# kuwt/edge_alignment

Measured on NVIDIA B200. Metric: frame-pair alignments/sec at 640x480, higher is better.
Workload: dtype f32+f64

## Files before the change

edge_alignment_b200/csrc/ea_preprocess.cu:

```cuda
#include <cstdlib>

#include "ea_internal.h"

namespace {

__device__ __forceinline__ int reflect101(int i, int n) {
  if (n == 1) return 0;
  while (i < 0 || i >= n) i = (i < 0) ? -i : 2 * n - 2 - i;
  return i;
}

template <typename D>
__global__ void __launch_bounds__(256) k_pyr_down(const uint8_t* __restrict__ src_bgr, const D* __restrict__ src_depth,
                                                  size_t src_frame_stride_px, const int32_t* __restrict__ src_slots,
                                                  uint8_t* __restrict__ dst_bgr, D* __restrict__ dst_depth,
                                                  const int32_t* __restrict__ dst_slots, int sw, int sh) {
  const int dw = sw >> 1, dh = sh >> 1;
  const int f = blockIdx.y;
  const size_t sbase = (src_slots ? size_t(src_slots[f]) : size_t(f)) * src_frame_stride_px;
  const size_t dbase = size_t(dst_slots[f]) * size_t(dw) * dh;
  for (int i = blockIdx.x * blockDim.x + threadIdx.x; i < dw * dh; i += gridDim.x * blockDim.x) {
    const int x = i % dw, y = i / dw;
    const uint8_t* p = src_bgr + (sbase + size_t(2 * y) * sw + 2 * x) * 3;
    const uint8_t* q = p + size_t(sw) * 3;
// ... 274 lines not shown
  const D* dep = depth + (src_slots ? size_t(src_slots[f]) : size_t(f)) * frame_stride_px;
  uint2* out = reinterpret_cast<uint2*>(pts + size_t(slot) * cap);
  const int nw = h * words;
  const int per = (nw + CP_THREADS - 1) / CP_THREADS;
  const int tid = threadIdx.x, lane = tid & 31, warp = tid >> 5;
  const int b = tid * per, e = min(b + per, nw);
  int cnt = 0;
  for (int i = b; i < e; ++i) cnt += __popc(bits[i]);
  int incl = cnt;
#pragma unroll
  for (int o = 1; o < 32; o <<= 1) { const int t = __shfl_up_sync(0xffffffffu, incl, o); if (lane >= o) incl += t; }
  if (lane == 31) warp_sums[warp] = incl;
  __syncthreads();
  if (warp == 0) {
    int v = warp_sums[lane];
    int s = v;
#pragma unroll
    for (int o = 1; o < 32; o <<= 1) { const int t = __shfl_up_sync(0xffffffffu, s, o); if (lane >= o) s += t; }
    warp_sums[lane] = s - v;
    if (lane == 31) total_s = s;
  }
  __syncthreads();
  int rank = warp_sums[warp] + incl - cnt;
  for (int i = b; i < e; ++i) {
    unsigned m = bits[i];
    const int y = i / words, xb = (i % words) * 32;
    while (m) {
      const int bit = __ffs(m) - 1;
      m &= m - 1;
      const int x = xb + bit;
      if (rank < cap) {
        float dz = float(dep[size_t(y) * w + x]);
        if (zero_to_one && dz == 0.0f) dz = depth_one;
        out[rank] = ea_pack_pixel_point(unsigned(x), unsigned(y), dz);
      }
      ++rank;
    }
  }
  if (tid == 0) {
    n_pts[slot * EA_MAX_LEVELS + level] = min(total_s, cap);
    overflow[slot * EA_MAX_LEVELS + level] = total_s > cap ? 1 : 0;
  }
}

__device__ __forceinline__ unsigned long long median3_bits64(unsigned long long a, unsigned long long b, unsigned long long c) {
  const unsigned long long s0 = a ^ b ^ c, s1 = (a & b) | (c & (a ^ b));
  const unsigned long long A0 = s0, B0 = s0 >> 1, C0 = s0 >> 2, A1 = s1, B1 = s1 >> 1, C1 = s1 >> 2;
  const unsigned long long lo = A0 ^ B0 ^ C0, carry = (A0 & B0) | (C0 & (A0 ^ B0));
  const unsigned long long t = A1 ^ B1, u = A1 & B1, v = C1 ^ carry, wv = C1 & carry;
  const unsigned long long m0 = t ^ v, tv = t & v;
  const unsigned long long ge1 = u | wv | tv, eq2 = u & wv;
  const unsigned long long m_ge3 = eq2 | (ge1 & m0);
  const unsigned long long m_eq2 = ge1 & ~eq2 & ~m0;
  return m_ge3 | (m_eq2 & lo);
}
__device__ __forceinline__ unsigned long long row_field64(const uint32_t* __restrict__ row, int wi, int words, int w) {
  const unsigned word = row[wi];
  const int nvalid = min(32, w - 32 * wi);
  const unsigned left = (wi > 0) ? (row[wi - 1] >> 31) : (word & 1u);
  unsigned right;
  if (nvalid == 32 && wi + 1 < words) right = row[wi + 1] & 1u;
  else right = (word >> (nvalid - 1)) & 1u;
  return (static_cast<unsigned long long>(word) << 1) | left | (static_cast<unsigned long long>(right) << (nvalid + 1));
}
__global__ void __launch_bounds__(256) k_median_bits(const __grid_constant__ EaPrepArgs A) {
  const int level = blockIdx.z;
  const EaPrepLevel& L = A.lv[level];
  const int idx = blockIdx.x * blockDim.x + threadIdx.x;
  if (idx >= L.h * L.words) return;
  const int slot = A.slots[blockIdx.y];
  const uint32_t* bits = L.edge_bits + size_t(slot) * L.h * L.words;
  const int y = idx / L.words, wi = idx % L.words;
  const unsigned long long f0 = row_field64(bits + size_t(max(y - 1, 0)) * L.words, wi, L.words, L.w);
  const unsigned long long f1 = row_field64(bits + size_t(y) * L.words, wi, L.words, L.w);
  const unsigned long long f2 = row_field64(bits + size_t(min(y + 1, L.h - 1)) * L.words, wi, L.words, L.w);
  const int nvalid = min(32, L.w - 32 * wi);
  unsigned m = unsigned(median3_bits64(f0, f1, f2));
  if (nvalid < 32) m &= (1u << nvalid) - 1u;
  L.med_bits[size_t(slot) * L.h * L.words + idx] = m;
}

#define DT_HV 62587
#define DT_DG 89738
#define DT_INF 0x3FFFFFFF
#define DT_DISTMAX (0xFFFFFFFFu - 89738u)

template <int P, bool BACKWARD>
__device__ __forceinline__ void dt_row_scan(int (&d)[P], const int (&cval)[P], int lane, int warp, int n_warps, int par,
                                            int (*tot)[32], int (*first)[32], int& left_bnd, int& right_bnd) {
  int dl[P];
  int run = DT_INF;
#pragma unroll
  for (int kk = 0; kk < P; ++kk) {
    const int k = BACKWARD ? (P - 1 - kk) : kk;
    run = min(cval[k], run + DT_HV);
    dl[k] = run;
  }
  const int pos = BACKWARD ? (31 - lane) : lane;
  const int stepP = DT_HV * P;
  int e = min(run, DT_INF) - stepP * pos;
#pragma unroll
  for (int o = 1; o < 32; o <<= 1) {
    const int t = BACKWARD ? __shfl_down_sync(0xffffffffu, e, o) : __shfl_up_sync(0xffffffffu, e, o);
    if (pos >= o) e = min(e, t);
  }
  const int out = e + stepP * pos;
  int carry_local = BACKWARD ? __shfl_down_sync(0xffffffffu, out, 1) : __shfl_up_sync(0xffffffffu, out, 1);
  if (pos == 0) carry_local = DT_INF;
  const int Lw = __shfl_sync(0xffffffffu, out, BACKWARD ? 0 : 31);
  const int f0 = __shfl_sync(0xffffffffu, BACKWARD ? dl[P - 1] : dl[0], BACKWARD ? 31 : 0);
  if (lane == 0) { tot[par][warp] = min(Lw, DT_INF); first[par][warp] = min(f0, DT_INF); }
  __syncthreads();
  const int wpos = BACKWARD ? (n_warps - 1 - warp) : warp;
  const int stepW = stepP * 32;
  int cand = DT_INF;
  if (lane < wpos) {
    const int src = BACKWARD ? (n_warps - 1 - lane) : lane;
    cand = tot[par][src] + stepW * (wpos - 1 - lane);
  }
  const int cw = min(__reduce_min_sync(0xffffffffu, cand), DT_INF);
#pragma unroll
  for (int kk = 0; kk < P; ++kk) {
    const int k = BACKWARD ? (P - 1 - kk) : kk;
    const int v = min(min(dl[k], carry_local + DT_HV * (kk + 1)), cw + DT_HV * (pos * P + kk + 1));
    d[k] = min(v, DT_INF);
  }
  const int out_w = min(min(Lw, cw + stepW), DT_INF);
  const int dn = BACKWARD ? warp - 1 : warp + 1;
  const int dn_first = (dn >= 0 && dn < n_warps) ? min(first[par][dn], out_w + DT_HV) : DT_INF;
  if (BACKWARD) { right_bnd = cw; left_bnd = dn_first; }
  else { left_bnd = cw; right_bnd = dn_first; }
}

template <int P, typename T>
__device__ __forceinline__ void dt_store_row(T* __restrict__ row, int x0, int w, const T (&v)[P], bool vec_ok) {
  if (vec_ok && x0 + P <= w) {
#pragma unroll
    for (int k = 0; k < P; k += 4) *reinterpret_cast<int4*>(row + x0 + k) = *reinterpret_cast<const int4*>(&v[k]);
  } else {
#pragma unroll
    for (int k = 0; k < P; ++k) if (x0 + k < w) row[x0 + k] = v[k];
  }
}
template <int P>
__device__ __forceinline__ void dt_load_row(const int* __restrict__ row, int x0, int w, int (&v)[P], bool vec_ok) {
  if (vec_ok && x0 + P <= w) {
#pragma unroll
    for (int k = 0; k < P; k += 4) *reinterpret_cast<int4*>(&v[k]) = *reinterpret_cast<const int4*>(row + x0 + k);
  } else {
#pragma unroll
    for (int k = 0; k < P; ++k) v[k] = (x0 + k < w) ? row[x0 + k] : DT_INF;
  }
}

template <int P>
__global__ void __launch_bounds__(1024) k_chamfer_dt(const __grid_constant__ EaPrepArgs A) {
  __shared__ int tot[2][32], first[2][32];
  __shared__ unsigned red[2][32];
  const int level = blockIdx.y;
  const EaPrepLevel& L = A.lv[level];
  const int w = L.w, h = L.h, words = L.words;
  const int slot = A.slots[blockIdx.x];
  const uint32_t* bits = (A.use_median ? L.med_bits : L.edge_bits) + size_t(slot) * h * words;
  float* gf = ea_dt_origin(L, slot);
  int* gi = reinterpret_cast<int*>(gf);
  const int pitch = L.dt_pitch;
  const int tid = threadIdx.x, lane = tid & 31, warp = tid >> 5;
  const int n_warps = ((w + P - 1) / P + 31) / 32;
  const bool warp_on = warp < n_warps;
  const int x0 = tid * P;
  const bool vec_ok = (P % 4 == 0) && ((w & 3) == 0);
  int d[P];
#pragma unroll
  for (int k = 0; k < P; ++k) d[k] = DT_INF;
  int left_bnd = DT_INF, right_bnd = DT_INF;
  int par = 0;
  unsigned ebits_next = (warp_on && x0 < w) ? bits[x0 >> 5] : 0u;
  for (int y = 0; y < h; ++y, par ^= 1) {
    if (!warp_on) { __syncthreads(); continue; }
    const unsigned ebits = ebits_next >> (x0 & 31);
    if (x0 < w && y + 1 < h) ebits_next = bits[size_t(y + 1) * words + (x0 >> 5)];
    int pl = __shfl_up_sync(0xffffffffu, d[P - 1], 1);
    int pr = __shfl_down_sync(0xffffffffu, d[0], 1);
    if (lane == 0) pl = left_bnd;
    if (lane == 31) pr = right_bnd;
    int cval[P];
#pragma unroll
    for (int k = 0; k < P; ++k) {
      const int a = (k == 0) ? pl : d[k - 1];
      const int c = (k == P - 1) ? pr : d[k + 1];
      int v = min(min(a, c) + DT_DG, d[k] + DT_HV);
      if ((ebits >> k) & 1u) v = 0;
      if (x0 + k >= w) v = DT_INF;
      cval[k] = min(v, DT_INF);
    }
    dt_row_scan<P, false>(d, cval, lane, warp, n_warps, par, tot, first, left_bnd, right_bnd);
#pragma unroll
    for (int k = 0; k < P; ++k) if (x0 + k >= w) d[k] = DT_INF;
    if (x0 < w) dt_store_row<P, int>(gi + size_t(y) * pitch, x0, w, d, vec_ok);
  }
#pragma unroll
  for (int k = 0; k < P; ++k) d[k] = DT_INF;
  left_bnd = DT_INF; right_bnd = DT_INF;
  unsigned vmax = 0, vmin = 0xFFFFFFFFu;
  int t_next[P];
#pragma unroll
  for (int k = 0; k < P; ++k) t_next[k] = DT_INF;
  if (warp_on && x0 < w) dt_load_row<P>(gi + size_t(h - 1) * pitch, x0, w, t_next, vec_ok);
  for (int y = h - 1; y >= 0; --y, par ^= 1) {
    if (!warp_on) { __syncthreads(); continue; }
    int t0[P];
#pragma unroll
    for (int k = 0; k < P; ++k) t0[k] = t_next[k];
    if (y > 0 && x0 < w) dt_load_row<P>(gi + size_t(y - 1) * pitch, x0, w, t_next, vec_ok);
    int pl = __shfl_up_sync(0xffffffffu, d[P - 1], 1);
    int pr = __shfl_down_sync(0xffffffffu, d[0], 1);
    if (lane == 0) pl = left_bnd;
    if (lane == 31) pr = right_bnd;
    int cval[P];
#pragma unroll
    for (int k = 0; k < P; ++k) {
      const int a = (k == 0) ? pl : d[k - 1];
      const int c = (k == P - 1) ? pr : d[k + 1];
      int v = min(t0[k], min(min(a, c) + DT_DG, d[k] + DT_HV));
      if (x0 + k >= w) v = DT_INF;
      cval[k] = min(v, DT_INF);
    }
    dt_row_scan<P, true>(d, cval, lane, warp, n_warps, par, tot, first, left_bnd, right_bnd);
    float outv[P];
#pragma unroll
    for (int k = 0; k < P; ++k) {
      outv[k] = 0.0f;
      if (x0 + k >= w) { d[k] = DT_INF; continue; }
      const unsigned t = (d[k] >= DT_INF) ? DT_DISTMAX : unsigned(d[k]);
      vmax = max(vmax, t); vmin = min(vmin, t);
      outv[k] = float(t) * (1.0f / 65536.0f);
    }
    if (x0 < w) dt_store_row<P, float>(gf + size_t(y) * pitch, x0, w, outv, vec_ok);
  }
  vmax = __reduce_max_sync(0xffffffffu, vmax);
  vmin = __reduce_min_sync(0xffffffffu, vmin);
  if (lane == 0) { red[0][warp] = vmin; red[1][warp] = vmax; }
  __syncthreads();
  if (tid == 0) {
    unsigned mn = 0xFFFFFFFFu, mx = 0;
    for (int i = 0; i < n_warps; ++i) { mn = min(mn, red[0][i]); mx = max(mx, red[1][i]); }
    A.dt_minmax[(slot * EA_MAX_LEVELS + level) * 2] = mn;
    A.dt_minmax[(slot * EA_MAX_LEVELS + level) * 2 + 1] = mx;
    float2 aff = make_float2(1.0f, 0.0f);
    if (A.dt_normalize != EA_NORM_NONE) {
      const double beta = (A.dt_normalize == EA_NORM_255) ? 255.0 : 1.0;
      const float fmn = float(mn) * (1.0f / 65536.0f), fmx = float(mx) * (1.0f / 65536.0f);
      const double range = double(fmx) - double(fmn);
      const double scale = beta * (range > 2.220446049250313e-16 ? 1.0 / range : 0.0);
      aff = make_float2(float(scale), float(0.0 - double(fmn) * scale));
    }
    A.dt_affine[slot * EA_MAX_LEVELS + level] = aff;
  }
}

#define DTW_PMAX 20
template <int P, bool BACKWARD, int SEG>
__device__ __forceinline__ void dtw_row_scan(int (&d)[P], const int (&cval)[P], const int lp) {
  static_assert(P % 4 == 0, "strip length must be a multiple of 4");
  int e[P];
#pragma unroll
  for (int kk = 0; kk < P; ++kk) e[kk] = cval[BACKWARD ? (P - 1 - kk) : kk] - DT_HV * kk;
  int m[P / 4];
#pragma unroll
  for (int g = 0; g < P / 4; ++g) m[g] = min(min(e[4 * g], e[4 * g + 1]), min(e[4 * g + 2], e[4 * g + 3]));
  int mt = m[0];
#pragma unroll
  for (int g = 1; g < P / 4; ++g) mt = min(mt, m[g]);
  const int run = min(mt + DT_HV * (P - 1), DT_INF);
  const int pos = BACKWARD ? (SEG - 1 - lp) : lp;
  constexpr int stepP = DT_HV * P;
  int s = run - stepP * pos;
#pragma unroll
  for (int o = 1; o < SEG; o <<= 1) {
    const int t = BACKWARD ? __shfl_down_sync(0xffffffffu, s, o, SEG) : __shfl_up_sync(0xffffffffu, s, o, SEG);
    if (pos >= o) s = min(s, t);
  }
  const int out = s + stepP * pos;
  int carry = BACKWARD ? __shfl_down_sync(0xffffffffu, out, 1, SEG) : __shfl_up_sync(0xffffffffu, out, 1, SEG);
  if (pos == 0) carry = DT_INF;
  carry = min(carry, DT_INF);
  int gp[P / 4];
  gp[0] = DT_INF;
#pragma unroll
  for (int g = 1; g < P / 4; ++g) gp[g] = min(gp[g - 1], m[g - 1]);
#pragma unroll
  for (int g = 0; g < P / 4; ++g) {
    int pm = gp[g];
#pragma unroll
    for (int i = 0; i < 4; ++i) {
      const int kk = 4 * g + i;
      pm = min(pm, e[kk]);
      const int v = min(pm, carry + DT_HV) + DT_HV * kk;
      d[BACKWARD ? (P - 1 - kk) : kk] = v;
    }
  }
}

#ifndef DTW_L2_AHEAD
#define DTW_L2_AHEAD 4
#endif
template <int P, bool FULL, int SEG>
__device__ __forceinline__ void dtw_level(const EaPrepArgs& A, const int level, const int lane) {
  const EaPrepLevel& L = A.lv[level];
  const int lp = lane % SEG;
  const int fi = int(blockIdx.x) * (32 / SEG) + lane / SEG;
  const bool frame_on = fi < A.n;
  const int slot = A.slots[frame_on ? fi : 0];
  const unsigned seg_mask = (0xffffffffu >> (32 - SEG)) << ((lane / SEG) * SEG);
  const int w = FULL ? SEG * P : L.w, h = L.h, words = L.words;
  const uint32_t* bits = (A.use_median ? L.med_bits : L.edge_bits) + size_t(slot) * h * words;
  float* gf = ea_dt_origin(L, slot);
  int* gi = reinterpret_cast<int*>(gf);
  const int pitch = L.dt_pitch;
  const int x0 = lp * P;
  const bool on = frame_on && x0 < w;
  const bool vec_ok = (P % 4 == 0) && ((w & 3) == 0);
  const int wi = x0 >> 5, sh = x0 & 31;
  const bool two = on && (wi + 1 < words);
  int d[P];
#pragma unroll
  for (int k = 0; k < P; ++k) d[k] = DT_INF;
  unsigned b0 = on ? bits[wi] : 0u, b1 = two ? bits[wi + 1] : 0u;
  for (int y = 0; y < h; ++y) {
    const unsigned ebits = __funnelshift_r(b0, b1, sh);
    if (y + DTW_L2_AHEAD < h && lp == 0) asm volatile("prefetch.global.L2 [%0];" ::"l"(bits + size_t(y + DTW_L2_AHEAD) * words));
    if (y + 1 < h) {
      b0 = on ? bits[size_t(y + 1) * words + wi] : 0u;
      b1 = two ? bits[size_t(y + 1) * words + wi + 1] : 0u;
    }
    int pl = __shfl_up_sync(0xffffffffu, d[P - 1], 1, SEG);
    int pr = __shfl_down_sync(0xffffffffu, d[0], 1, SEG);
    if (lp == 0) pl = DT_INF;
    if (lp == SEG - 1) pr = DT_INF;
    int cval[P];
#pragma unroll
    for (int k = 0; k < P; ++k) {
      const int a = (k == 0) ? pl : d[k - 1];
      const int c = (k == P - 1) ? pr : d[k + 1];
      int v = min(min(a, c) + DT_DG, d[k] + DT_HV);
      if ((ebits >> k) & 1u) v = 0;
      if (!FULL && x0 + k >= w) v = DT_INF;
      cval[k] = v;
    }
    dtw_row_scan<P, false, SEG>(d, cval, lp);
#pragma unroll
    for (int k = 0; k < P; ++k) if (!FULL && x0 + k >= w) d[k] = DT_INF;
    if (on) dt_store_row<P, int>(gi + size_t(y) * pitch, x0, w, d, vec_ok);
  }
#pragma unroll
  for (int k = 0; k < P; ++k) d[k] = DT_INF;
  unsigned vmax = 0, vmin = 0xFFFFFFFFu;
  int t_next[P];
#pragma unroll
  for (int k = 0; k < P; ++k) t_next[k] = DT_INF;
  __syncwarp();
  if (on) dt_load_row<P>(gi + size_t(h - 1) * pitch, x0, w, t_next, vec_ok);
  for (int y = h - 1; y >= 0; --y) {
    int t0[P];
#pragma unroll
    for (int k = 0; k < P; ++k) t0[k] = t_next[k];
    if (y > 0 && on) dt_load_row<P>(gi + size_t(y - 1) * pitch, x0, w, t_next, vec_ok);
    if (y >= DTW_L2_AHEAD && frame_on && lp * 32 < w)
      asm volatile("prefetch.global.L2 [%0];" ::"l"(gi + size_t(y - DTW_L2_AHEAD) * pitch + lp * 32));
    int pl = __shfl_up_sync(0xffffffffu, d[P - 1], 1, SEG);
    int pr = __shfl_down_sync(0xffffffffu, d[0], 1, SEG);
    if (lp == 0) pl = DT_INF;
    if (lp == SEG - 1) pr = DT_INF;
    int cval[P];
#pragma unroll
    for (int k = 0; k < P; ++k) {
      const int a = (k == 0) ? pl : d[k - 1];
      const int c = (k == P - 1) ? pr : d[k + 1];
      int v = min(t0[k], min(min(a, c) + DT_DG, d[k] + DT_HV));
      if (!FULL && x0 + k >= w) v = DT_INF;
      cval[k] = v;
    }
    dtw_row_scan<P, true, SEG>(d, cval, lp);
    float outv[P];
#pragma unroll
    for (int k = 0; k < P; ++k) {
      outv[k] = 0.0f;
      if (!FULL && x0 + k >= w) { d[k] = DT_INF; continue; }
      const unsigned t = (d[k] >= DT_INF) ? DT_DISTMAX : unsigned(d[k]);
      vmax = max(vmax, t); vmin = min(vmin, t);
      outv[k] = float(t) * (1.0f / 65536.0f);
    }
    const int copies = (y == 0 || y == h - 1) ? 1 + EA_DT_PAD : 1;
    const int ystep = (y == 0) ? -1 : 1;
    const bool last_strip = on && (x0 + P >= w);
    float edge_r = 0.0f;
    if (last_strip) {
#pragma unroll
      for (int k = 0; k < P; ++k) if (x0 + k == w - 1) edge_r = outv[k];
    }
    for (int c = 0; c < copies; ++c) {
      float* row = gf + (ptrdiff_t(y) + ptrdiff_t(c) * ystep) * pitch;
      if (on) dt_store_row<P, float>(row, x0, w, outv, vec_ok);
      if (lp == 0 && frame_on) *reinterpret_cast<float4*>(row - EA_DT_PAD) = make_float4(outv[0], outv[0], outv[0], outv[0]);
      if (last_strip) for (int x = w; x < pitch - EA_DT_PAD; ++x) row[x] = edge_r;
    }
    if (h == 1 && y == 0) {
      for (int c = 1; c <= EA_DT_PAD; ++c) {
        float* row = gf + ptrdiff_t(c) * pitch;
        if (on) dt_store_row<P, float>(row, x0, w, outv, vec_ok);
        if (lp == 0 && frame_on) *reinterpret_cast<float4*>(row - EA_DT_PAD) = make_float4(outv[0], outv[0], outv[0], outv[0]);
        if (last_strip) for (int x = w; x < pitch - EA_DT_PAD; ++x) row[x] = edge_r;
      }
    }
  }
  const unsigned mx = __reduce_max_sync(seg_mask, vmax);
  const unsigned mn = __reduce_min_sync(seg_mask, vmin);
  if (lp == 0 && frame_on) {
    A.dt_minmax[(slot * EA_MAX_LEVELS + level) * 2] = mn;
    A.dt_minmax[(slot * EA_MAX_LEVELS + level) * 2 + 1] = mx;
    float2 aff = make_float2(1.0f, 0.0f);
    if (A.dt_normalize != EA_NORM_NONE) {
      const double beta = (A.dt_normalize == EA_NORM_255) ? 255.0 : 1.0;
      const float fmn = float(mn) * (1.0f / 65536.0f), fmx = float(mx) * (1.0f / 65536.0f);
      const double range = double(fmx) - double(fmn);
      const double scale = beta * (range > 2.220446049250313e-16 ? 1.0 / range : 0.0);
      aff = make_float2(float(scale), float(0.0 - double(fmn) * scale));
    }
    A.dt_affine[slot * EA_MAX_LEVELS + level] = aff;
  }
}

__host__ __device__ __forceinline__ int dtw_seg(int w) {
  return w == 16 * DTW_PMAX ? 16 : w == 8 * DTW_PMAX ? 8 : w == 4 * DTW_PMAX ? 4 : 32;
}
__global__ void __launch_bounds__(32) k_chamfer_dt_warp(const __grid_constant__ EaPrepArgs A) {
  const int level = blockIdx.y, lane = threadIdx.x;
  const int w = A.lv[level].w;
  const int seg = dtw_seg(w);
  if (int(blockIdx.x) * (32 / seg) >= A.n) return;
  const int per = (w + 31) / 32;
  if (seg == 16) dtw_level<DTW_PMAX, true, 16>(A, level, lane);
  else if (seg == 8) dtw_level<DTW_PMAX, true, 8>(A, level, lane);
  else if (seg == 4) dtw_level<DTW_PMAX, true, 4>(A, level, lane);
  else if (per <= 8) { if (w == 256) dtw_level<8, true, 32>(A, level, lane); else dtw_level<8, false, 32>(A, level, lane); }
  else if (per <= 12) { if (w == 384) dtw_level<12, true, 32>(A, level, lane); else dtw_level<12, false, 32>(A, level, lane); }
  else { if (w == 32 * DTW_PMAX) dtw_level<DTW_PMAX, true, 32>(A, level, lane); else dtw_level<DTW_PMAX, false, 32>(A, level, lane); }
}

__global__ void __launch_bounds__(256) k_dt_normalized_copy(const float* __restrict__ origin, int pitch, const float2* __restrict__ affine,
                                                            int w, int h, float* __restrict__ out) {
  const float2 a = *affine;
  for (int i = blockIdx.x * blockDim.x + threadIdx.x; i < w * h; i += gridDim.x * blockDim.x)
    out[i] = __fadd_rn(__fmul_rn(origin[size_t(i / w) * pitch + (i % w)], a.x), a.y);
}

__global__ void __launch_bounds__(256) k_dt_import(const float* __restrict__ src, float* __restrict__ origin, int w, int h, int pitch) {
  const int n = pitch * (h + 2 * EA_DT_PAD);
  for (int i = blockIdx.x * blockDim.x + threadIdx.x; i < n; i += gridDim.x * blockDim.x) {
    const int py = i / pitch - EA_DT_PAD, px = i % pitch - EA_DT_PAD;
    origin[ptrdiff_t(py) * pitch + px] = src[size_t(min(max(py, 0), h - 1)) * w + min(max(px, 0), w - 1)];
  }
}
__global__ void __launch_bounds__(256) k_dt_fill_pad(float* __restrict__ pool, size_t slot_floats, const int32_t* __restrict__ slots,
                                                     int w, int h, int pitch) {
  float* origin = pool + size_t(slots[blockIdx.y]) * slot_floats + size_t(EA_DT_PAD) * pitch + EA_DT_PAD;
  const int n = pitch * (h + 2 * EA_DT_PAD);
  for (int i = blockIdx.x * blockDim.x + threadIdx.x; i < n; i += gridDim.x * blockDim.x) {
    const int py = i / pitch - EA_DT_PAD, px = i % pitch - EA_DT_PAD;
    if (py >= 0 && py < h && px >= 0 && px < w) continue;
    origin[ptrdiff_t(py) * pitch + px] = origin[size_t(min(max(py, 0), h - 1)) * pitch + min(max(px, 0), w - 1)];
  }
}

__global__ void __launch_bounds__(256) k_unpack_mask(const uint32_t* __restrict__ bits, int w, int h, int words, int median,
                                                     uint8_t* __restrict__ out) {
  for (int i = blockIdx.x * blockDim.x + threadIdx.x; i < w * h; i += gridDim.x * blockDim.x) {
    const int x = i % w, y = i / w;
    int edge;
    if (!median) edge = (bits[size_t(y) * words + (x >> 5)] >> (x & 31)) & 1;
    else {
      int cnt = 0;
      for (int dy = -1; dy <= 1; ++dy)
        for (int dx = -1; dx <= 1; ++dx) {
          const int xx = min(max(x + dx, 0), w - 1), yy = min(max(y + dy, 0), h - 1);
          cnt += (bits[size_t(yy) * words + (xx >> 5)] >> (xx & 31)) & 1;
        }
      edge = cnt >= 5;
    }
    out[i] = edge ? 0 : 255;
  }
}

}

static bool edge_kernel_fuses_pyramid(const EaPrepArgs& A, int l) {
  if (l + 1 >= A.n_levels || A.edge_detector != EA_EDGE_LAPLACIAN) return false;
  const EaPrepLevel& L = A.lv[l];
  const EaPrepLevel& N = A.lv[l + 1];
  static const int env_fuse = getenv("EA_PYR_FUSE") ? atoi(getenv("EA_PYR_FUSE")) : 1;
  return env_fuse && (L.w & 3) == 0 && L.w >= 8 && L.h >= 4 && (N.w & 3) == 0 && (reinterpret_cast<uintptr_t>(N.bgr) & 3) == 0;
}

template <typename D>
static cudaError_t launch_edges_and_points(const EaPrepArgs& A, cudaStream_t stream, int& nl) {
  const bool want_ref = (A.roles & EA_ROLE_REF) != 0;
  const size_t px0 = size_t(A.lv[0].w) * A.lv[0].h;
  const D* in_depth = static_cast<const D*>(A.in_depth);
  for (int l = 0; l < A.n_levels; ++l) {
    const EaPrepLevel& L = A.lv[l];
    const size_t pxl = size_t(L.w) * L.h;
    if (l > 0 && !edge_kernel_fuses_pyramid(A, l - 1)) {
      const EaPrepLevel& S = A.lv[l - 1];
      const uint8_t* sb = (l == 1) ? A.in_bgr : S.bgr;
      const D* sd = want_ref ? ((l == 1) ? in_depth : static_cast<const D*>(S.depth)) : nullptr;
      const size_t sstride = (l == 1) ? px0 : size_t(S.w) * S.h;
      const bool vec4 = ((L.w & 3) == 0) && ((reinterpret_cast<uintptr_t>(sb) & 7) == 0) && ((reinterpret_cast<uintptr_t>(L.bgr) & 3) == 0);
      if (vec4) {
        dim3 grid(unsigned((pxl / 4 + 255) / 256), unsigned(A.n));
        k_pyr_down4<D><<<grid, 256, 0, stream>>>(sb, sd, sstride, (l == 1) ? nullptr : A.slots, L.bgr, static_cast<D*>(L.depth), A.slots, S.w, S.h);
      } else {
        dim3 grid(unsigned((pxl + 255) / 256), unsigned(A.n));
        k_pyr_down<D><<<grid, 256, 0, stream>>>(sb, sd, sstride, (l == 1) ? nullptr : A.slots, L.bgr, static_cast<D*>(L.depth), A.slots, S.w, S.h);
      }
      ++nl;
    }
    const uint8_t* b = (l == 0) ? A.in_bgr : L.bgr;
    const D* d = want_ref ? ((l == 0) ? in_depth : static_cast<const D*>(L.depth)) : nullptr;
    const int32_t* ss = (l == 0) ? nullptr : A.slots;
    if (A.edge_detector != EA_EDGE_LAPLACIAN) {
      int k = 0;
      cudaError_t ce = ea_launch_canny_level(A, l, b, d, pxl, l != 0, A.canny, A.scratch, stream, &k);
      nl += k - 1;
      if (ce != cudaSuccess) return ce;
    } else if ((L.w & 3) == 0 && L.w >= 8 && L.h >= 4) {
      const bool fuse = edge_kernel_fuses_pyramid(A, l);
      uint8_t* nb = fuse ? A.lv[l + 1].bgr : nullptr;
      D* nd = (fuse && want_ref) ? static_cast<D*>(A.lv[l + 1].depth) : nullptr;
      if ((L.w % 128) != 0 && (L.w % 128) <= 64) {
        dim3 grid(unsigned((L.w + 63) / 64), unsigned((L.h + E2_TH - 1) / E2_TH), unsigned(A.n));
        if (want_ref) k_edge_mask2<D, 64, true><<<grid, 64, 0, stream>>>(b, d, pxl, ss, A.slots, L.edge_bits, L.ref_bits, L.w, L.h, L.words, A.grad_threshold, A.zero_to_one, nb, nd);
        else k_edge_mask2<D, 64, false><<<grid, 64, 0, stream>>>(b, d, pxl, ss, A.slots, L.edge_bits, nullptr, L.w, L.h, L.words, A.grad_threshold, A.zero_to_one, nb, nd);
      } else {
        dim3 grid(unsigned((L.w + E2_TW - 1) / E2_TW), unsigned((L.h + E2_TH - 1) / E2_TH), unsigned(A.n));
        if (want_ref) k_edge_mask2<D, E2_TW, true><<<grid, E2_TW, 0, stream>>>(b, d, pxl, ss, A.slots, L.edge_bits, L.ref_bits, L.w, L.h, L.words, A.grad_threshold, A.zero_to_one, nb, nd);
        else k_edge_mask2<D, E2_TW, false><<<grid, E2_TW, 0, stream>>>(b, d, pxl, ss, A.slots, L.edge_bits, nullptr, L.w, L.h, L.words, A.grad_threshold, A.zero_to_one, nb, nd);
      }
    } else {
      dim3 grid(unsigned((L.w + ET_W - 1) / ET_W), unsigned((L.h + ET_H - 1) / ET_H), unsigned(A.n));
      k_edge_mask<D><<<grid, dim3(ET_W, ET_H), 0, stream>>>(b, d, pxl, ss, A.slots, L.edge_bits, want_ref ? L.ref_bits : nullptr, L.w, L.h, L.words, A.grad_threshold, A.zero_to_one);
    }
    ++nl;
    if (want_ref && A.in_mask) {
      k_mask_ref_bits<<<dim3(unsigned((L.h * L.words + 255) / 256), unsigned(A.n)), 256, 0, stream>>>(L.ref_bits, A.slots, A.in_mask, A.lv[0].w, A.lv[0].h, L.w, L.h, L.words, l, 0);
      ++nl;
    }
    if (A.in_now_mask) {
      k_mask_ref_bits<<<dim3(unsigned((L.h * L.words + 255) / 256), unsigned(A.n)), 256, 0, stream>>>(L.edge_bits, A.slots, A.in_now_mask, A.lv[0].w, A.lv[0].h, L.w, L.h, L.words, l, 1);
      ++nl;
    }
    if (want_ref) {
      k_compact<D><<<A.n, CP_THREADS, 0, stream>>>(L.ref_bits, d, pxl, ss, A.slots, L.pts, A.n_pts, l, A.overflow, L.w, L.h, L.words, L.cap, A.zero_to_one, A.depth_one);
      ++nl;
    }
  }
  return cudaGetLastError();
}

static cudaError_t launch_front(const EaPrepArgs& A, cudaStream_t stream, int& nl) {
  const bool want_now = (A.roles & EA_ROLE_NOW) != 0;
  cudaError_t pe = (A.depth_type == 1) ? launch_edges_and_points<float>(A, stream, nl) : launch_edges_and_points<uint16_t>(A, stream, nl);
  if (pe != cudaSuccess) return pe;
  if (want_now && A.dt_kind != EA_DT_EXACT && A.use_median) {
    const EaPrepLevel& L0 = A.lv[0];
    dim3 grid(unsigned((L0.h * L0.words + 255) / 256), unsigned(A.n), unsigned(A.n_levels));
    k_median_bits<<<grid, 256, 0, stream>>>(A);
    ++nl;
  }
  return cudaGetLastError();
}
static cudaError_t launch_dt(const EaPrepArgs& A, cudaStream_t stream, int& nl) {
  if (A.dt_kind == EA_DT_EXACT) {
    for (int l = 0; l < A.n_levels; ++l) {
      cudaError_t ee = ea_launch_exact_edt_level(A, l, A.scratch, stream, &nl);
      if (ee != cudaSuccess) return ee;
    }
    return cudaGetLastError();
  }
  const EaPrepLevel& L0 = A.lv[0];
  static const int env_block = getenv("EA_DT_BLOCK") ? atoi(getenv("EA_DT_BLOCK")) : 0;
  if (L0.w <= 32 * DTW_PMAX && !env_block) {
    k_chamfer_dt_warp<<<dim3(unsigned(A.n), unsigned(A.n_levels)), 32, 0, stream>>>(A);
    ++nl;
    return cudaGetLastError();
  }
  int P = (L0.w <= 4096) ? 4 : 8;
  if (const char* e = getenv("EA_DT_P")) { const int v = atoi(e); if ((v == 2 || v == 4 || v == 8) && v > P) P = v; }
  const int threads = (((L0.w + P - 1) / P + 31) / 32) * 32;
  if (threads > 1024) return cudaErrorInvalidValue;
  dim3 grid(unsigned(A.n), unsigned(A.n_levels));
  if (P == 2) k_chamfer_dt<2><<<grid, threads, 0, stream>>>(A);
  else if (P == 4) k_chamfer_dt<4><<<grid, threads, 0, stream>>>(A);
  else k_chamfer_dt<8><<<grid, threads, 0, stream>>>(A);
  ++nl;
  for (int l = 0; l < A.n_levels; ++l) { ea_launch_dt_fill_pad(A.lv[l], A.slots, A.n, stream); ++nl; }
  return cudaGetLastError();
}
static EaPrepArgs prep_slice(const EaPrepArgs& A, int f0, int n) {
  EaPrepArgs S = A;
  const size_t px0 = size_t(A.lv[0].w) * A.lv[0].h;
  S.n = n; S.slots = A.slots + f0;
  S.in_bgr = A.in_bgr + size_t(f0) * px0 * 3;
  if (A.in_depth) S.in_depth = static_cast<const char*>(A.in_depth) + size_t(f0) * px0 * (A.depth_type == 1 ? 4 : 2);
  if (A.in_mask) S.in_mask = A.in_mask + size_t(f0) * px0;
  if (A.in_now_mask) S.in_now_mask = A.in_now_mask + size_t(f0) * px0;
  return S;
}

cudaError_t ea_launch_preprocess(const EaPrepArgs& A, int sm_count, cudaStream_t stream, int* launches, const EaPrepPipe* pipe) {
  int nl = 0;
  const bool want_ref = (A.roles & EA_ROLE_REF) != 0, want_now = (A.roles & EA_ROLE_NOW) != 0;
  if (want_ref && !A.in_depth) return cudaErrorInvalidValue;
  static const int env_split = getenv("EA_PREP_SPLIT") ? atoi(getenv("EA_PREP_SPLIT")) : 8;
  const bool split = env_split > 0 && pipe && pipe->ready && want_now && A.edge_detector == EA_EDGE_LAPLACIAN && A.dt_kind != EA_DT_EXACT &&
                     A.lv[0].w <= 32 * DTW_PMAX && A.n >= env_split * sm_count;
  cudaError_t e = cudaSuccess;
  if (!split) {
    e = launch_front(A, stream, nl);
    if (e == cudaSuccess && want_now) e = launch_dt(A, stream, nl);
  } else {
    static const int env_parts = getenv("EA_PREP_PARTS") ? atoi(getenv("EA_PREP_PARTS")) : 2;
    const int K = env_parts < 2 ? 2 : env_parts > EA_PREP_MAX_PARTS ? EA_PREP_MAX_PARTS : env_parts;
    int forked = 0;
    for (int k = 0; k < K && e == cudaSuccess; ++k) {
      const int f0 = int((long long)A.n * k / K), f1 = int((long long)A.n * (k + 1) / K);
      const EaPrepArgs H = prep_slice(A, f0, f1 - f0);
      e = launch_front(H, stream, nl);
      if (e != cudaSuccess) break;
      e = cudaEventRecord(pipe->ev_front[k], stream);
      if (e == cudaSuccess) e = cudaStreamWaitEvent(pipe->aux[k], pipe->ev_front[k], 0);
      if (e != cudaSuccess) break;
      forked = k + 1;
      e = launch_dt(H, pipe->aux[k], nl);
    }
    for (int k = 0; k < forked; ++k) {
      cudaError_t je = cudaEventRecord(pipe->ev_dt[k], pipe->aux[k]);
      if (je == cudaSuccess) je = cudaStreamWaitEvent(stream, pipe->ev_dt[k], 0);
      if (e == cudaSuccess) e = je;
    }
  }
  (void)sm_count;
  if (launches) *launches = nl;
  return e != cudaSuccess ? e : cudaGetLastError();
}

cudaError_t ea_launch_dt_normalized_copy(const float* origin, int pitch, const float2* affine, int w, int h, float* out, cudaStream_t stream) {
  k_dt_normalized_copy<<<(w * h + 255) / 256, 256, 0, stream>>>(origin, pitch, affine, w, h, out);
  return cudaGetLastError();
}
cudaError_t ea_launch_dt_import(const float* src, float* origin, int w, int h, int pitch, cudaStream_t stream) {
  const int n = pitch * (h + 2 * EA_DT_PAD);
  k_dt_import<<<(n + 255) / 256, 256, 0, stream>>>(src, origin, w, h, pitch);
  return cudaGetLastError();
}
cudaError_t ea_launch_dt_fill_pad(const EaPrepLevel& L, const int32_t* d_slots, int n, cudaStream_t stream) {
  const int tot = L.dt_pitch * (L.h + 2 * EA_DT_PAD);
  k_dt_fill_pad<<<dim3(unsigned(std::min((tot + 255) / 256, 1024)), unsigned(n)), 256, 0, stream>>>(L.dt, L.dt_slot, d_slots, L.w, L.h, L.dt_pitch);
  return cudaGetLastError();
}

cudaError_t ea_launch_unpack_mask(const uint32_t* bits, int w, int h, int words, int median, uint8_t* out, cudaStream_t stream) {
  k_unpack_mask<<<(w * h + 255) / 256, 256, 0, stream>>>(bits, w, h, words, median, out);
  return cudaGetLastError();
}
```

Measured before the change: 117,800.

## Fuse 3x3 median bit filter into warp chamfer DT row loop

When the warp-level chamfer DT kernel is used, the separate k_median_bits launch is skipped. The DT kernel instead reads raw edge bits and computes the 3x3 median on the fly from a rolling three-row window of 64-bit fields, including left and right neighbour bits and edge replication. This removes a kernel launch and the write and re-read of the median bit buffer, at the cost of extra loads and bit arithmetic per row inside the serial DT loop.

```diff
diff --git a/edge_alignment_b200/csrc/ea_preprocess.cu b/edge_alignment_b200/csrc/ea_preprocess.cu
--- a/edge_alignment_b200/csrc/ea_preprocess.cu
+++ b/edge_alignment_b200/csrc/ea_preprocess.cu
@@ -600,6 +600,18 @@
   }
 }
 
+__device__ __forceinline__ uint3 dtw_mask_words(const uint32_t* __restrict__ row, int wi, int sh, bool on, bool two) {
+  return make_uint3((on && sh == 0 && wi > 0) ? row[wi - 1] : 0u, on ? row[wi] : 0u, two ? row[wi + 1] : 0u);
+}
+template <int P>
+__device__ __forceinline__ unsigned long long dtw_mask_field(uint3 r, int wi, int sh, int e) {
+  const unsigned long long W = (static_cast<unsigned long long>(r.z) << 32) | r.y;
+  const unsigned left = sh > 0 ? (r.y >> (sh - 1)) & 1u : wi > 0 ? r.x >> 31 : r.y & 1u;
+  unsigned long long f = ((W >> sh) << 1) | left;
+  if (unsigned(e - 1) < unsigned(P)) f |= ((f >> e) & 1ull) << (e + 1);
+  return f;
+}
+
 #ifndef DTW_L2_AHEAD
 #define DTW_L2_AHEAD 4
 #endif
@@ -612,7 +624,7 @@
   const int slot = A.slots[frame_on ? fi : 0];
   const unsigned seg_mask = (0xffffffffu >> (32 - SEG)) << ((lane / SEG) * SEG);
   const int w = FULL ? SEG * P : L.w, h = L.h, words = L.words;
-  const uint32_t* bits = (A.use_median ? L.med_bits : L.edge_bits) + size_t(slot) * h * words;
+  const uint32_t* bits = L.edge_bits + size_t(slot) * h * words;
   float* gf = ea_dt_origin(L, slot);
   int* gi = reinterpret_cast<int*>(gf);
   const int pitch = L.dt_pitch;
@@ -624,14 +636,15 @@
   int d[P];
 #pragma unroll
   for (int k = 0; k < P; ++k) d[k] = DT_INF;
-  unsigned b0 = on ? bits[wi] : 0u, b1 = two ? bits[wi + 1] : 0u;
+  const bool med = A.use_median != 0;
+  uint3 nx = dtw_mask_words(bits + size_t(min(1, h - 1)) * words, wi, sh, on, two);
+  unsigned long long fa = dtw_mask_field<P>(dtw_mask_words(bits, wi, sh, on, two), wi, sh, w - x0), fb = fa;
   for (int y = 0; y < h; ++y) {
-    const unsigned ebits = __funnelshift_r(b0, b1, sh);
+    const unsigned long long fc = dtw_mask_field<P>(nx, wi, sh, w - x0);
     if (y + DTW_L2_AHEAD < h && lp == 0) asm volatile("prefetch.global.L2 [%0];" ::"l"(bits + size_t(y + DTW_L2_AHEAD) * words));
-    if (y + 1 < h) {
-      b0 = on ? bits[size_t(y + 1) * words + wi] : 0u;
-      b1 = two ? bits[size_t(y + 1) * words + wi + 1] : 0u;
-    }
+    if (y + 1 < h) nx = dtw_mask_words(bits + size_t(min(y + 2, h - 1)) * words, wi, sh, on, two);
+    const unsigned ebits = med ? unsigned(median3_bits64(fa, fb, fc)) : unsigned(fb >> 1);
+    fa = fb; fb = fc;
     int pl = __shfl_up_sync(0xffffffffu, d[P - 1], 1, SEG);
     int pr = __shfl_down_sync(0xffffffffu, d[0], 1, SEG);
     if (lp == 0) pl = DT_INF;
@@ -865,11 +878,15 @@
   return cudaGetLastError();
 }
 
+static bool dt_uses_warp_kernel(const EaPrepArgs& A) {
+  static const int env_block = getenv("EA_DT_BLOCK") ? atoi(getenv("EA_DT_BLOCK")) : 0;
+  return A.lv[0].w <= 32 * DTW_PMAX && !env_block;
+}
 static cudaError_t launch_front(const EaPrepArgs& A, cudaStream_t stream, int& nl) {
   const bool want_now = (A.roles & EA_ROLE_NOW) != 0;
   cudaError_t pe = (A.depth_type == 1) ? launch_edges_and_points<float>(A, stream, nl) : launch_edges_and_points<uint16_t>(A, stream, nl);
   if (pe != cudaSuccess) return pe;
-  if (want_now && A.dt_kind != EA_DT_EXACT && A.use_median) {
+  if (want_now && A.dt_kind != EA_DT_EXACT && A.use_median && !dt_uses_warp_kernel(A)) {
     const EaPrepLevel& L0 = A.lv[0];
     dim3 grid(unsigned((L0.h * L0.words + 255) / 256), unsigned(A.n), unsigned(A.n_levels));
     k_median_bits<<<grid, 256, 0, stream>>>(A);
@@ -886,8 +903,7 @@
     return cudaGetLastError();
   }
   const EaPrepLevel& L0 = A.lv[0];
-  static const int env_block = getenv("EA_DT_BLOCK") ? atoi(getenv("EA_DT_BLOCK")) : 0;
-  if (L0.w <= 32 * DTW_PMAX && !env_block) {
+  if (dt_uses_warp_kernel(A)) {
     k_chamfer_dt_warp<<<dim3(unsigned(A.n), unsigned(A.n_levels)), 32, 0, stream>>>(A);
     ++nl;
     return cudaGetLastError();
```

Measured after the change: 119,800, median of 6. +1.8%, better.

## Checkpoint forward distance-transform rows and recompute them per segment in backward pass

Applied to the files above, without the earlier changes.

The forward DT sweep now stores its integer row to global memory only every DTW_CK-th row, as a checkpoint. The backward sweep walks segments of DTW_CK rows from the bottom. For each segment it reloads the checkpoint, recomputes the forward rows into registers, then runs the backward rows from them, while prefetching the next segment's edge bits and checkpoint. This removes most of the intermediate int row writes and reads to global memory. In exchange the forward sweep is computed twice for most rows and more registers are held (t[DTW_CK][P]), which could hurt occupancy.

```diff
diff --git a/edge_alignment_b200/csrc/ea_preprocess.cu b/edge_alignment_b200/csrc/ea_preprocess.cu
--- a/edge_alignment_b200/csrc/ea_preprocess.cu
+++ b/edge_alignment_b200/csrc/ea_preprocess.cu
@@ -603,6 +603,102 @@
 #ifndef DTW_L2_AHEAD
 #define DTW_L2_AHEAD 4
 #endif
+#ifndef DTW_CK
+#define DTW_CK 4
+#endif
+
+template <int P, bool FULL, int SEG>
+__device__ __forceinline__ void dtw_fwd_row(int (&d)[P], const unsigned ebits, const int lp, const int x0, const int w) {
+  int pl = __shfl_up_sync(0xffffffffu, d[P - 1], 1, SEG);
+  int pr = __shfl_down_sync(0xffffffffu, d[0], 1, SEG);
+  if (lp == 0) pl = DT_INF;
+  if (lp == SEG - 1) pr = DT_INF;
+  int cval[P];
+#pragma unroll
+  for (int k = 0; k < P; ++k) {
+    const int a = (k == 0) ? pl : d[k - 1];
+    const int c = (k == P - 1) ? pr : d[k + 1];
+    int v = min(min(a, c) + DT_DG, d[k] + DT_HV);
+    if ((ebits >> k) & 1u) v = 0;
+    if (!FULL && x0 + k >= w) v = DT_INF;
+    cval[k] = v;
+  }
+  dtw_row_scan<P, false, SEG>(d, cval, lp);
+#pragma unroll
+  for (int k = 0; k < P; ++k) if (!FULL && x0 + k >= w) d[k] = DT_INF;
+}
+
+template <int P, bool FULL, int SEG>
+__device__ __forceinline__ void dtw_bwd_row(int (&d)[P], const int (&t0)[P], const int lp, const int x0, const int w) {
+  int pl = __shfl_up_sync(0xffffffffu, d[P - 1], 1, SEG);
+  int pr = __shfl_down_sync(0xffffffffu, d[0], 1, SEG);
+  if (lp == 0) pl = DT_INF;
+  if (lp == SEG - 1) pr = DT_INF;
+  int cval[P];
+#pragma unroll
+  for (int k = 0; k < P; ++k) {
+    const int a = (k == 0) ? pl : d[k - 1];
+    const int c = (k == P - 1) ? pr : d[k + 1];
+    int v = min(t0[k], min(min(a, c) + DT_DG, d[k] + DT_HV));
+    if (!FULL && x0 + k >= w) v = DT_INF;
+    cval[k] = v;
+  }
+  dtw_row_scan<P, true, SEG>(d, cval, lp);
+}
+
+template <int P, bool FULL>
+__device__ __forceinline__ void dtw_store_out(int (&d)[P], const int lp, const int x0, const int w, const int y, const int h,
+                                              float* __restrict__ gf, const int pitch, const bool on, const bool frame_on,
+                                              const bool vec_ok, unsigned& vmin, unsigned& vmax) {
+  float outv[P];
+#pragma unroll
+  for (int k = 0; k < P; ++k) {
+    outv[k] = 0.0f;
+    if (!FULL && x0 + k >= w) { d[k] = DT_INF; continue; }
+    const unsigned t = (d[k] >= DT_INF) ? DT_DISTMAX : unsigned(d[k]);
+    vmax = max(vmax, t); vmin = min(vmin, t);
+    outv[k] = float(t) * (1.0f / 65536.0f);
+  }
+  const int copies = (y == 0 || y == h - 1) ? 1 + EA_DT_PAD : 1;
+  const int ystep = (y == 0) ? -1 : 1;
+  const bool last_strip = on && (x0 + P >= w);
+  float edge_r = 0.0f;
+  if (last_strip) {
+#pragma unroll
+    for (int k = 0; k < P; ++k) if (x0 + k == w - 1) edge_r = outv[k];
+  }
+  for (int c = 0; c < copies; ++c) {
+    float* row = gf + (ptrdiff_t(y) + ptrdiff_t(c) * ystep) * pitch;
+    if (on) dt_store_row<P, float>(row, x0, w, outv, vec_ok);
+    if (lp == 0 && frame_on) *reinterpret_cast<float4*>(row - EA_DT_PAD) = make_float4(outv[0], outv[0], outv[0], outv[0]);
+    if (last_strip) for (int x = w; x < pitch - EA_DT_PAD; ++x) row[x] = edge_r;
+  }
+  if (h == 1 && y == 0) {
+    for (int c = 1; c <= EA_DT_PAD; ++c) {
+      float* row = gf + ptrdiff_t(c) * pitch;
+      if (on) dt_store_row<P, float>(row, x0, w, outv, vec_ok);
+      if (lp == 0 && frame_on) *reinterpret_cast<float4*>(row - EA_DT_PAD) = make_float4(outv[0], outv[0], outv[0], outv[0]);
+      if (last_strip) for (int x = w; x < pitch - EA_DT_PAD; ++x) row[x] = edge_r;
+    }
+  }
+}
+
+template <int P>
+__device__ __forceinline__ void dtw_fetch_segment(const uint32_t* __restrict__ bits, const int* __restrict__ gi, const int pitch,
+                                                  const int words, const int w, const int h, const int y0, const int wi, const int x0,
+                                                  const bool on, const bool two, const bool vec_ok, unsigned (&m0)[DTW_CK],
+                                                  unsigned (&m1)[DTW_CK], int (&ck)[P]) {
+#pragma unroll
+  for (int r = 0; r < DTW_CK; ++r) {
+    const bool in = y0 + r < h;
+    m0[r] = (on && in) ? bits[size_t(y0 + r) * words + wi] : 0u;
+    m1[r] = (two && in) ? bits[size_t(y0 + r) * words + wi + 1] : 0u;
+  }
+#pragma unroll
+  for (int k = 0; k < P; ++k) ck[k] = DT_INF;
+  if (y0 > 0 && on) dt_load_row<P>(gi + size_t(y0 - 1) * pitch, x0, w, ck, vec_ok);
+}
+
 template <int P, bool FULL, int SEG>
 __device__ __forceinline__ void dtw_level(const EaPrepArgs& A, const int level, const int lane) {
   const EaPrepLevel& L = A.lv[level];
@@ -624,91 +720,46 @@
   int d[P];
 #pragma unroll
   for (int k = 0; k < P; ++k) d[k] = DT_INF;
+  const int n_seg = (h + DTW_CK - 1) / DTW_CK;
+  const int h_fwd = (n_seg - 1) * DTW_CK;
   unsigned b0 = on ? bits[wi] : 0u, b1 = two ? bits[wi + 1] : 0u;
-  for (int y = 0; y < h; ++y) {
+  for (int y = 0; y < h_fwd; ++y) {
     const unsigned ebits = __funnelshift_r(b0, b1, sh);
     if (y + DTW_L2_AHEAD < h && lp == 0) asm volatile("prefetch.global.L2 [%0];" ::"l"(bits + size_t(y + DTW_L2_AHEAD) * words));
-    if (y + 1 < h) {
+    if (y + 1 < h_fwd) {
       b0 = on ? bits[size_t(y + 1) * words + wi] : 0u;
       b1 = two ? bits[size_t(y + 1) * words + wi + 1] : 0u;
     }
-    int pl = __shfl_up_sync(0xffffffffu, d[P - 1], 1, SEG);
-    int pr = __shfl_down_sync(0xffffffffu, d[0], 1, SEG);
-    if (lp == 0) pl = DT_INF;
-    if (lp == SEG - 1) pr = DT_INF;
-    int cval[P];
-#pragma unroll
-    for (int k = 0; k < P; ++k) {
-      const int a = (k == 0) ? pl : d[k - 1];
-      const int c = (k == P - 1) ? pr : d[k + 1];
-      int v = min(min(a, c) + DT_DG, d[k] + DT_HV);
-      if ((ebits >> k) & 1u) v = 0;
-      if (!FULL && x0 + k >= w) v = DT_INF;
-      cval[k] = v;
-    }
-    dtw_row_scan<P, false, SEG>(d, cval, lp);
-#pragma unroll
-    for (int k = 0; k < P; ++k) if (!FULL && x0 + k >= w) d[k] = DT_INF;
-    if (on) dt_store_row<P, int>(gi + size_t(y) * pitch, x0, w, d, vec_ok);
+    dtw_fwd_row<P, FULL, SEG>(d, ebits, lp, x0, w);
+    if (on && y % DTW_CK == DTW_CK - 1) dt_store_row<P, int>(gi + size_t(y) * pitch, x0, w, d, vec_ok);
   }
 #pragma unroll
   for (int k = 0; k < P; ++k) d[k] = DT_INF;
   unsigned vmax = 0, vmin = 0xFFFFFFFFu;
-  int t_next[P];
-#pragma unroll
-  for (int k = 0; k < P; ++k) t_next[k] = DT_INF;
-  __syncwarp();
-  if (on) dt_load_row<P>(gi + size_t(h - 1) * pitch, x0, w, t_next, vec_ok);
-  for (int y = h - 1; y >= 0; --y) {
-    int t0[P];
-#pragma unroll
-    for (int k = 0; k < P; ++k) t0[k] = t_next[k];
-    if (y > 0 && on) dt_load_row<P>(gi + size_t(y - 1) * pitch, x0, w, t_next, vec_ok);
-    if (y >= DTW_L2_AHEAD && frame_on && lp * 32 < w)
-      asm volatile("prefetch.global.L2 [%0];" ::"l"(gi + size_t(y - DTW_L2_AHEAD) * pitch + lp * 32));
-    int pl = __shfl_up_sync(0xffffffffu, d[P - 1], 1, SEG);
-    int pr = __shfl_down_sync(0xffffffffu, d[0], 1, SEG);
-    if (lp == 0) pl = DT_INF;
-    if (lp == SEG - 1) pr = DT_INF;
-    int cval[P];
-#pragma unroll
-    for (int k = 0; k < P; ++k) {
-      const int a = (k == 0) ? pl : d[k - 1];
-      const int c = (k == P - 1) ? pr : d[k + 1];
-      int v = min(t0[k], min(min(a, c) + DT_DG, d[k] + DT_HV));
-      if (!FULL && x0 + k >= w) v = DT_INF;
-      cval[k] = v;
-    }
-    dtw_row_scan<P, true, SEG>(d, cval, lp);
-    float outv[P];
-#pragma unroll
-    for (int k = 0; k < P; ++k) {
-      outv[k] = 0.0f;
-      if (!FULL && x0 + k >= w) { d[k] = DT_INF; continue; }
-      const unsigned t = (d[k] >= DT_INF) ? DT_DISTMAX : unsigned(d[k]);
-      vmax = max(vmax, t); vmin = min(vmin, t);
-      outv[k] = float(t) * (1.0f / 65536.0f);
-    }
-    const int copies = (y == 0 || y == h - 1) ? 1 + EA_DT_PAD : 1;
-    const int ystep = (y == 0) ? -1 : 1;
-    const bool last_strip = on && (x0 + P >= w);
-    float edge_r = 0.0f;
-    if (last_strip) {
-#pragma unroll
-      for (int k = 0; k < P; ++k) if (x0 + k == w - 1) edge_r = outv[k];
-    }
-    for (int c = 0; c < copies; ++c) {
-      float* row = gf + (ptrdiff_t(y) + ptrdiff_t(c) * ystep) * pitch;
-      if (on) dt_store_row<P, float>(row, x0, w, outv, vec_ok);
-      if (lp == 0 && frame_on) *reinterpret_cast<float4*>(row - EA_DT_PAD) = make_float4(outv[0], outv[0], outv[0], outv[0]);
-      if (last_strip) for (int x = w; x < pitch - EA_DT_PAD; ++x) row[x] = edge_r;
-    }
-    if (h == 1 && y == 0) {
-      for (int c = 1; c <= EA_DT_PAD; ++c) {
-        float* row = gf + ptrdiff_t(c) * pitch;
-        if (on) dt_store_row<P, float>(row, x0, w, outv, vec_ok);
-        if (lp == 0 && frame_on) *reinterpret_cast<float4*>(row - EA_DT_PAD) = make_float4(outv[0], outv[0], outv[0], outv[0]);
-        if (last_strip) for (int x = w; x < pitch - EA_DT_PAD; ++x) row[x] = edge_r;
+  unsigned m0[DTW_CK], m1[DTW_CK];
+  int ck[P];
+  dtw_fetch_segment<P>(bits, gi, pitch, words, w, h, h_fwd, wi, x0, on, two, vec_ok, m0, m1, ck);
+  for (int s = n_seg - 1; s >= 0; --s) {
+    const int y0 = s * DTW_CK, rows = min(DTW_CK, h - y0);
+    int f[P];
+    unsigned eb[DTW_CK];
+#pragma unroll
+    for (int k = 0; k < P; ++k) f[k] = ck[k];
+#pragma unroll
+    for (int r = 0; r < DTW_CK; ++r) eb[r] = __funnelshift_r(m0[r], m1[r], sh);
+    if (s > 0) dtw_fetch_segment<P>(bits, gi, pitch, words, w, h, y0 - DTW_CK, wi, x0, on, two, vec_ok, m0, m1, ck);
+    int t[DTW_CK][P];
+#pragma unroll
+    for (int r = 0; r < DTW_CK; ++r) {
+      if (r < rows) dtw_fwd_row<P, FULL, SEG>(f, eb[r], lp, x0, w);
+#pragma unroll
+      for (int k = 0; k < P; ++k) t[r][k] = f[k];
+    }
+#pragma unroll
+    for (int r = DTW_CK - 1; r >= 0; --r) {
+      if (r < rows) {
+        dtw_bwd_row<P, FULL, SEG>(d, t[r], lp, x0, w);
+        dtw_store_out<P, FULL>(d, lp, x0, w, y0 + r, h, gf, pitch, on, frame_on, vec_ok, vmin, vmax);
       }
     }
   }
```

After: 117,900 before, 113,500 after, median of 6. 0.963x the previous value.
